# LuxGraph/Lux

Hardware: NVIDIA H100
Metric: MTEPS (higher is better)
Workload: dtype f32

## Files before the change

lux_b200/csrc/api.cu:

```cuda
#include <cub/cub.cuh>
#include <stdarg.h>
#include <stdlib.h>
#include <string.h>
#include <algorithm>
#include <type_traits>
#include <new>

#include "build.cuh"
#include "cf.cuh"
#include "pull.cuh"
#include "panel.cuh"
#include "seg.cuh"
#include "push.cuh"
#include "runtime.cuh"
#include <thrust/iterator/counting_iterator.h>

using namespace luxb;

enum class AppRun : uint8_t { kIterations, kConvergence, kEntry };
static constexpr char kBcRun[] = "luxb_bc_run";

struct AppInfo {
  const char* name;
  AppRun run;
  const char* entry;
  bool weights;
  bool dist_labels;
  uint32_t vbytes;
  bool check;
  bool settable;
};
static constexpr AppInfo kApps[] = {
    {"pagerank",                        AppRun::kIterations,  nullptr,          false,  false, 4,        false, true},
    {"connected components",            AppRun::kConvergence, nullptr,          false,  false, 4,        true,  true},
    {"SSSP",                            AppRun::kConvergence, nullptr,          false,  false, 4,        true,  true},
    {"col_filter",                      AppRun::kIterations,  nullptr,          true,   false, 4 * kCfK, false, true},
    {"weighted SSSP",                   AppRun::kConvergence, nullptr,          true,   true,  4,        true,  true},
    {"betweenness centrality",          AppRun::kEntry,       kBcRun,           false,  false, 8,        false, true},
    {"weighted betweenness centrality", AppRun::kEntry,       kBcRun,           true,   true,  8,        false, true},
    {"triangle counting",               AppRun::kEntry,       "luxb_tc_run",    false,  false, 8,        false, false},
    {"k-core decomposition",            AppRun::kEntry,       "luxb_kcore_run", false,  false, 4,        true,  true},
    {"k-truss decomposition",           AppRun::kEntry,       "luxb_truss_run", false,  false, 4,        true,  false},
};
static constexpr int kNumApps = sizeof(kApps) / sizeof(kApps[0]);
static_assert(kNumApps == LUXB_TRUSS + 1, "one row per luxb_app");
static const AppInfo& app_of(const luxb_graph* g) { return kApps[g->cfg.app]; }

static const char* const kPhaseName[12] = {"pull_tile", "fixup", "refresh", "rechunk", "barrier", "panel", "combine", "pack+push", "pull/bcast", "cold_hub", "bc_sigma", "bc_delta"};
static void pt_mark(luxb_graph* g, int tag) {
  PhaseTimer& pt = g->pt;
  if (!pt.on) return;
  cudaEvent_t e;
  cudaEventCreate(&e);
  cudaEventRecord(e, g->stream);
  pt.ev.push_back(e);
  pt.tag.push_back(tag);
}
static void pt_print(luxb_graph* g) {
  if (g->pt.on && g->pt.cnt) {
    char line[1024];
    const bool bc = app_of(g).entry == kBcRun;
    int n = snprintf(line, sizeof(line), "[luxb rank %d] phase means over %ld %s:", g->cfg.rank, g->pt.cnt, bc ? "sources" : "iterations");
    double sum = 0;
    for (int k = bc ? 10 : 0; k < (bc ? 12 : 10); ++k) {
      n += snprintf(line + n, sizeof(line) - n, " %s %.3f ms;", kPhaseName[k], g->pt.sum[k] / g->pt.cnt);
      sum += g->pt.sum[k] / g->pt.cnt;
    }
    snprintf(line + n, sizeof(line) - n, " sum %.3f ms\n", sum);
    fputs(line, stderr);
  }
}

static void pt_flush(luxb_graph* g) {
  PhaseTimer& pt = g->pt;
  if (!pt.on || pt.ev.empty()) return;
  cudaStreamSynchronize(g->stream);
  for (size_t i = 1; i < pt.ev.size(); ++i) {
    if (pt.tag[i] < 0) continue;
    float ms = 0;
    cudaEventElapsedTime(&ms, pt.ev[i - 1], pt.ev[i]);
    pt.sum[pt.tag[i]] += ms;
    if (pt.tag[i] == (app_of(g).entry == kBcRun ? 10 : 0)) pt.cnt++;
  }
  for (cudaEvent_t e : pt.ev) cudaEventDestroy(e);
  pt.ev.clear();
  pt.tag.clear();
}


namespace luxb {
static thread_local char g_err[1024] = "";
void set_error(const char* fmt, ...) {
  va_list ap;
  va_start(ap, fmt);
  vsnprintf(g_err, sizeof(g_err), fmt, ap);
  va_end(ap);
}
}

#define LUXB_ARG(cond, ...)             \
  do {                                  \
    if (!(cond)) {                      \
      set_error(__VA_ARGS__);           \
      return LUXB_ERR_ARG;              \
    }                                   \
  } while (0)

#define LUXB_NCCL(expr)                                                                              \
  do {                                                                                               \
    ncclResult_t _r = (expr);                                                                        \
    if (_r != ncclSuccess) {                                                                         \
      set_error("NCCL error %s at %s:%d: %s", #expr, __FILE__, __LINE__, nccl().GetErrorString(_r)); \
      return LUXB_ERR_COMM;                                                                          \
    }                                                                                                \
  } while (0)

#define LUXB_PULL_SHAPES(X) X(0, 7, 8, 2) X(1, 9, 8, 2) X(2, 7, 16, 2)
#define LUXB_DECL_SHAPE(id, ipt, warps, stages) using PullShape##id = PullShape<ipt, warps, stages>;
LUXB_PULL_SHAPES(LUXB_DECL_SHAPE)
// ... 785 lines not shown
      uint32_t zero = 0;
      if (start < g->nv)
        LUXB_CUDA(cudaMemcpyAsync(lab + start, &zero, 4, cudaMemcpyHostToDevice, g->stream));
    }
    LUXB_CUDA(cudaGetLastError());
  }
  if (g->n_part)
    LUXB_CUDA(cudaMemcpyAsync(g->d_cur, lab + g->row_left, (size_t)g->n_part * 4, cudaMemcpyDeviceToDevice, g->stream));
  LUXB_CUDA(cudaStreamSynchronize(g->stream));
  g->stats.last_active = 0;
  for (int p = 0; p < g->P; ++p) g->stats.last_active += g->h_hdr[2 * p + 1];
  g->stats.last_frontier_type = g->h_hdr[2 * g->cfg.rank];
  return 0;
}

static constexpr double kColdSplitWindowMB = 12.0;
static int set_l2_persisting_window(luxb_graph* g, void* base, size_t bytes) {
  if (!g->sweep.l2_persist) return 0;
  int max_persist = 0, max_window = 0;
  LUXB_CUDA(cudaDeviceGetAttribute(&max_persist, cudaDevAttrMaxPersistingL2CacheSize, g->cfg.device));
  LUXB_CUDA(cudaDeviceGetAttribute(&max_window, cudaDevAttrMaxAccessPolicyWindowSize, g->cfg.device));
  if (max_persist <= 0 || max_window <= 0) return 0;
  if (g->sweep.l2_window_mb >= 0) bytes = std::min<size_t>(bytes, (size_t)(g->sweep.l2_window_mb * 1e6));
  else if (g->cs_on) bytes = std::min<size_t>(bytes, (size_t)(kColdSplitWindowMB * 1e6));
  size_t persist = std::min<size_t>((size_t)max_persist, bytes);
  LUXB_CUDA(cudaDeviceSetLimit(cudaLimitPersistingL2CacheSize, persist));
  cudaStreamAttrValue attr{};
  attr.accessPolicyWindow.base_ptr = base;
  attr.accessPolicyWindow.num_bytes = std::min<size_t>(bytes, (size_t)max_window);
  attr.accessPolicyWindow.hitRatio = (float)std::min(1.0, (double)persist / (double)attr.accessPolicyWindow.num_bytes);
  attr.accessPolicyWindow.hitProp = cudaAccessPropertyPersisting;
  attr.accessPolicyWindow.missProp = cudaAccessPropertyStreaming;
  LUXB_CUDA(cudaStreamSetAttribute(g->stream, cudaStreamAttributeAccessPolicyWindow, &attr));
  if (g->cfg.verbose) printf("L2 persisting window: %zu bytes (device max persisting %d, max window %d)\n", persist, max_persist, max_window);
  return 0;
}

static constexpr double kColdSplitMinShare = 0.05;
static constexpr uint64_t kSplitMinEdges = 1ull << 24;

static bool split_may_run(const luxb_graph* g) {
  const SweepSettings& s = g->sweep;
  return s.seg && s.sb != 0 && !g->cfg.zero_copy_edges && (s.sb > 0 || g->e_part >= kSplitMinEdges);
}

static int build_hot_layout(luxb_graph* g, bool compact_cold) {
  g->hot_n = 0;
  g->packed = false;
  g->cold_z = false;
  uint64_t h_max = (uint64_t)(g->sweep.hot_mb * 1e6 / 4.0);
  if (h_max == 0 || g->nv < 2 || (uint64_t)g->nv >= 0xFFFFFFFFull - h_max) return 0;
  if (h_max > g->nv) h_max = g->nv;
  const int grid = g->num_sms * 8;
  const uint32_t cap = 4096;
  DevTmp tmp;
  unsigned long long* d_hist = nullptr;
  LUXB_TRY(tmp.alloc(&d_hist, cap + 1));
  LUXB_CUDA(cudaMemsetAsync(d_hist, 0, (cap + 1) * 8, g->stream));
  degree_hist_kernel<<<grid, 256, 0, g->stream>>>(g->d_deg, g->nv, cap, d_hist);
  std::vector<unsigned long long> hist(cap + 1);
  LUXB_CUDA(cudaMemcpyAsync(hist.data(), d_hist, (cap + 1) * 8, cudaMemcpyDeviceToHost, g->stream));
  LUXB_CUDA(cudaStreamSynchronize(g->stream));
  uint64_t above = 0;
  uint32_t tau = cap + 1;
  for (uint32_t d = cap; d >= 2; --d) {
    if (above + hist[d] > h_max) break;
// ... 88 lines not shown
    if (g->n_part)
      pack_list_cold_kernel<<<grid, 256, 0, g->stream>>>(d_cflag, d_crank, g->row_left, g->n_part, g->cold_off[me], g->d_pack_list + nh_me);
    LUXB_CUDA(cudaGetLastError());
    g->packed = true;
  }
  gather_map_hot_kernel<<<grid, 256, 0, g->stream>>>(d_map, g->d_hot_order, H);
  LUXB_TRY(edge_alloc(g, &g->d_src_gather, g->e_part + 8));
  LUXB_CUDA(cudaMemsetAsync(g->d_src_gather, 0, (g->e_part + 8) * 4, g->stream));
  remap_src_kernel<<<grid, 256, 0, g->stream>>>(g->d_src, g->e_part, d_map, g->d_src_gather);
  LUXB_CUDA(cudaGetLastError());
  LUXB_CUDA(cudaStreamSynchronize(g->stream));
  g->hot_n = H;
  return 0;
}

static int allgather_slices(luxb_graph* g, void* replica, size_t elem_bytes);
static void resolve_sweep_settings(SweepSettings& s);
static int build_seg_sweep(luxb_graph* g);
static int pagerank_publish(luxb_graph* g, float* x_new);
static int wait_cold_exchange(luxb_graph* g);
static int bc_alloc(luxb_graph* g);
static int tc_build(luxb_graph* g);
static int kcore_build(luxb_graph* g);
static int truss_build(luxb_graph* g);

static int build_gather_side(luxb_graph* g, bool compact_cold, bool streams) {
  LUXB_TRY(gmalloc(g, &g->d_deg, g->nv));
  LUXB_CUDA(cudaMemsetAsync(g->d_deg, 0, (size_t)g->nv * 4, g->stream));
  hist_src_kernel<<<g->num_sms * 8, 256, 0, g->stream>>>(g->d_src, g->e_part, g->d_deg);
  LUXB_CUDA(cudaGetLastError());
  if (g->P > 1) LUXB_NCCL(nccl().AllReduce(g->d_deg, g->d_deg, g->nv, ncclUint32, ncclSum, g->comm, g->stream));
  LUXB_TRY(build_hot_layout(g, compact_cold));
  if (streams) LUXB_TRY(build_seg_sweep(g));
  if (g->hot_n) {
    const uint64_t z_len = (uint64_t)g->hot_n + (g->cold_z ? g->cold_n : 0) + 65536;
    LUXB_TRY(gmalloc(g, (uint32_t**)&g->d_hot, z_len));
    LUXB_CUDA(cudaMemsetAsync(g->d_hot, 0, z_len * 4, g->stream));
    LUXB_TRY(set_l2_persisting_window(g, g->d_hot, (size_t)g->hot_n * 4));
  }
  return 0;
}

int luxb_init(luxb_graph* g) {
  LUXB_ARG(g != nullptr, "graph is NULL");
  if (g->inited) { set_error("luxb_init called twice"); return LUXB_ERR_STATE; }
  if (g->P > 1 && !g->comm) { set_error("luxb_init: nranks > 1 needs luxb_comm_init first"); return LUXB_ERR_STATE; }
  LUXB_CUDA(cudaSetDevice(g->cfg.device));
  resolve_sweep_settings(g->sweep);
  const int grid = g->num_sms * 8;
  switch (g->cfg.app) {
    case LUXB_PAGERANK: {
      LUXB_TRY(build_gather_side(g, true, true));
      for (int k = 0; k < 2; ++k) LUXB_TRY(gmalloc(g, (float**)&g->d_val[k], (uint64_t)g->nv + 64));
      pr_init_kernel<<<grid, 256, 0, g->stream>>>(g->d_deg, g->nv, (float*)g->d_val[0]);
      LUXB_CUDA(cudaMemsetAsync(g->d_val[1], 0, (size_t)g->nv * 4, g->stream));
      if (g->packed) {
        g->xt_hot_chunk = ((((uint64_t)g->hot_n + g->P - 1) / g->P) + 31) & ~31ull;
        g->xt_cold_chunk = ((((uint64_t)g->cold_n + g->P - 1) / g->P) + 31) & ~31ull;
        const uint64_t xt_len = (g->xt_hot_chunk + g->xt_cold_chunk) * g->P;
        for (int k = 0; k < 2; ++k) {
          LUXB_TRY(gmalloc(g, &g->d_xt[k], xt_len));
          LUXB_CUDA(cudaMemsetAsync(g->d_xt[k], 0, xt_len * 4, g->stream));
        }
      }
      LUXB_CUDA(cudaGetLastError());
      LUXB_TRY(pagerank_publish(g, (float*)g->d_val[0]));
// ... 109 lines not shown
  return 0;
}

static int kt_begin(luxb_graph* g) {
  if (!g->kernel_timing) return 0;
  if (g->kt_used + 2 > g->kt_events.size()) {
    cudaEvent_t e0, e1;
    LUXB_CUDA(cudaEventCreate(&e0));
    LUXB_CUDA(cudaEventCreate(&e1));
    g->kt_events.push_back(e0);
    g->kt_events.push_back(e1);
  }
  LUXB_CUDA(cudaEventRecord(g->kt_events[g->kt_used], g->stream));
  return 0;
}
static int kt_end(luxb_graph* g) {
  if (!g->kernel_timing) return 0;
  LUXB_CUDA(cudaEventRecord(g->kt_events[g->kt_used + 1], g->stream));
  g->kt_used += 2;
  return 0;
}

template <class Prog>
static void fill_fixup_args(PullArgs<Prog>& a, const FixupScratch& f) {
  a.head_partial = reinterpret_cast<typename Prog::Acc*>(f.d_head);
  a.tail_partial = reinterpret_cast<typename Prog::Acc*>(f.d_tail);
  a.carry = reinterpret_cast<typename Prog::Wide*>(f.d_carry);
  a.carry_flag = f.d_carry_flag;
  a.block_agg = reinterpret_cast<typename Prog::Wide*>(f.d_block_agg);
  a.block_flag = f.d_block_flag;
}

template <class Prog>
static int launch_fixup(luxb_graph* g, const PullArgs<Prog>& a, FixupScratch& f, const uint2* piece_slot = nullptr) {
  if (a.n_tiles <= 1) return 0;
  if (g->fused_fixup) {
    if (!f.d_chain) {
      LUXB_TRY(gmalloc(g, &f.d_chain, 4ull * f.n_fix_blocks + 4));
      LUXB_CUDA(cudaMemsetAsync(f.d_chain, 0, (4ull * f.n_fix_blocks + 4) * 8, g->stream));
      f.chain_epoch = 0;
    }
    FixupChain<Prog> ch;
    ch.value = f.d_chain;
    ch.status = f.d_chain + 2ull * f.n_fix_blocks;
    ch.ticket = f.d_chain + 4ull * f.n_fix_blocks;
    ch.n_blocks = f.n_fix_blocks;
    ch.epoch = ++f.chain_epoch;
    if (f.chain_epoch >= 0x3FFFFFF0u) {
      LUXB_CUDA(cudaMemsetAsync(f.d_chain, 0, (4ull * f.n_fix_blocks + 4) * 8, g->stream));
      f.chain_epoch = ch.epoch = 1;
    }
    pull_fixup_fused_kernel<Prog><<<f.n_fix_blocks, kFixBlock, 0, g->stream>>>(a, ch, piece_slot);
    LUXB_CUDA(cudaGetLastError());
    g->stats.kernel_launches++;
    return 0;
  }
  pull_fixup_scan_kernel<Prog><<<f.n_fix_blocks, kFixBlock, 0, g->stream>>>(a);
  pull_fixup_blocks_kernel<Prog><<<1, 1024, 0, g->stream>>>(a, f.n_fix_blocks);
  pull_fixup_apply_kernel<Prog><<<f.n_fix_blocks, kFixBlock, 0, g->stream>>>(a, piece_slot);
  LUXB_CUDA(cudaGetLastError());
  g->stats.kernel_launches += 3;
  return 0;
}

template <class Prog>
static int launch_pull(luxb_graph* g, PullLayout& L, const uint32_t* src, const typename Prog::Vertex* x_nat,
                       const typename Prog::Vertex* x_cold, const typename Prog::Vertex* x_hot, uint32_t hot_n,
                       typename Prog::Vertex* out_local, const typename Prog::Params& prm, const uint32_t* hub_bits = nullptr,
                       bool timed = true) {
  if (L.n_tiles == 0) return 0;
  PullArgs<Prog> a{};
  a.row_end = L.d_row_end;
  a.row_end32 = L.d_row_end32;
  a.src = src;
  a.x_nat = x_nat;
  a.n_part = L.n_vtx;
  a.e_part = L.e_cnt;
  a.row_left = g->row_left;
  a.x_old = x_cold;
  a.x_hot = x_hot;
  a.hot_n = hot_n;
  a.out = out_local;
  a.tile_v = L.d_tile_v;
  a.n_tiles = L.n_tiles;
  fill_fixup_args(a, L.fix);
  a.tile_counter = reinterpret_cast<uint32_t*>(g->d_counters + 2);
  LUXB_CUDA(cudaMemsetAsync(a.tile_counter, 0, 4, g->stream));
  a.prm = prm;
  a.hub_bits = hub_bits;
  a.raw_out = 0;
  if constexpr (Prog::kWeighted) a.weight = g->d_weight;
  if (timed) LUXB_TRY(kt_begin(g));
// ... 26 lines not shown
static const SegShapeInfo kSegPanelInfo[] = {LUXB_SEG_PANEL_SHAPES(LUXB_PSHAPE_INFO)};
static const int kNumSegMain = sizeof(kSegMainInfo) / sizeof(SegShapeInfo);
static const int kNumSegPanel = sizeof(kSegPanelInfo) / sizeof(SegShapeInfo);

static int env_int(const char* name, int dflt) {
  const char* e = getenv(name);
  return e ? atoi(e) : dflt;
}

static double env_double(const char* name, double dflt) {
  const char* e = getenv(name);
  return e ? atof(e) : dflt;
}

static void resolve_sweep_settings(SweepSettings& s) {
  s = SweepSettings();
  if (const char* e = getenv("LUXB_SWEEP")) s.seg = strcmp(e, "merge") != 0;
  auto shape = [](const char* name, int dflt, int n) { const int v = env_int(name, dflt); return v < 0 || v >= n ? 0 : v; };
  s.main_shape = shape("LUXB_SEG_MAIN_SHAPE", s.main_shape, kNumSegMain);
  s.panel_shape = shape("LUXB_SEG_PANEL_SHAPE", s.panel_shape, kNumSegPanel);
  s.cs_shape = shape("LUXB_CS_SHAPE", s.main_shape, kNumSegMain);
  s.sb = env_int("LUXB_SB", s.sb);
  const int tab = kSegPanelInfo[s.panel_shape].tab;
  s.sb_bs = std::min<uint32_t>((uint32_t)std::max(4, env_int("LUXB_SB_BS", tab)) & ~3u, (uint32_t)tab);
  s.sb_blocks = (uint32_t)std::min(std::max(env_int("LUXB_SB_BLOCKS", (int)s.sb_blocks), 1), kPanelMaxBlocks);
  s.sb_min_indeg = (uint32_t)std::max(env_int("LUXB_SB_MIN_INDEG", (int)s.sb_min_indeg), 1);
  s.sb_tier = env_int("LUXB_SB_TIER", s.sb_tier);
  s.sb_slot_edges = env_double("LUXB_SB_SLOT_EDGES", s.sb_slot_edges);
  s.cs = env_int("LUXB_CS", s.cs);
  s.cs_seg_mb = env_double("LUXB_CS_SEG_MB", s.cs_seg_mb);
  s.hot_mb = env_double("LUXB_HOT_MB", s.hot_mb);
  s.l2_persist = env_int("LUXB_L2_PERSIST", 1) != 0;
  s.l2_window_mb = env_double("LUXB_L2_WINDOW_MB", s.l2_window_mb);
}

extern "C++" {
template <class Word, class In>
static int build_seg_stream(luxb_graph* g, PullLayout& L, const uint64_t* d_row_end, uint32_t n_vtx, const In* d_ids, uint64_t e_cnt,
                            StreamBlocks& blk, uint32_t stage_edges, uint32_t piece, bool want_empty, const uint32_t* hub_bits,
                            uint32_t* super_end, bool slots = false, uint32_t slot_base = 0) {
  const int grid = g->num_sms * 8;
  DevTmp tmp;
  L = PullLayout();
  L.n_vtx = n_vtx;
  L.e_cnt = e_cnt;
  uint64_t words = 0, pads_total = 0;
  for (uint32_t b = 0; b < blk.n_blocks; ++b) {
    const uint64_t eb = blk.ebase[b + 1] - blk.ebase[b];
    const uint64_t pad = stage_edges - eb % stage_edges;
    blk.wbase[b] = words;
    blk.hshift[b] = pads_total;
    words += eb + pad;
    pads_total += pad;
    if (super_end) super_end[b] = (uint32_t)(words / stage_edges);
  }
  blk.wbase[blk.n_blocks] = words;
  blk.hshift[blk.n_blocks] = pads_total;
  LUXB_ARG(words / piece < 0xFFFFFFF0ull && words / stage_edges < 0xFFFFFFF0ull, "stream too large");
  L.n_words = words;
  L.n_stages = (uint32_t)(words / stage_edges);
  L.n_tiles = (uint32_t)(words / piece);
  uint32_t *d_flag = nullptr, *d_rank = nullptr;
  LUXB_TRY(tmp.alloc(&d_flag, (uint64_t)n_vtx + 1));
  LUXB_TRY(tmp.alloc(&d_rank, (uint64_t)n_vtx + 1));
  nonempty_flag_kernel<<<grid, 256, 0, g->stream>>>(d_row_end, n_vtx, d_flag);
  LUXB_CUDA(cudaMemsetAsync(d_flag + n_vtx, 0, 4, g->stream));
// ... 324 lines not shown
  g->stats.panel_edges = e_cov0;
  g->stats.panel_hubs = Nh;
  g->stats.panel_blocks = NB0;
  g->stats.cold_hub_edges = e_cold;
  g->stats.cold_hub_segments = S;
  g->stats.tier_blocks = NB - NB0;
  g->stats.tier_slots = NV - (uint64_t)NB0 * Nh;
  g->stats.tier_edges = e_cov - e_cov0;
  if (g->cfg.verbose) {
    printf("[luxb rank %d] source-blocked sweep: %u hub destinations (in-degree >= %u) x %u blocks of %u hot sources, + %u tier blocks "
           "(%llu slots, %llu edges); panel %llu edges (%.1f %%), cold-hub %llu edges (%u segments of %u values), main %llu edges\n",
           g->cfg.rank, Nh, st.sb_min_indeg, NB0, bs, NB - NB0, (unsigned long long)(NV - (uint64_t)NB0 * Nh), (unsigned long long)(e_cov - e_cov0),
           (unsigned long long)e_cov, 100.0 * e_cov / g->e_part, (unsigned long long)e_cold, S, cs.seg, (unsigned long long)e_main);
    printf("[luxb rank %d] (group, hub) pairs with edges / all: tier 0 %u / %llu, tiers %u / %llu, cold segments %u / %llu\n", g->cfg.rank,
           kind_slots[1], (unsigned long long)NB0 * Nh, kind_slots[2] - kind_slots[1], (unsigned long long)(NV - (uint64_t)NB0 * Nh),
           kind_slots[3] - kind_slots[2], (unsigned long long)Nh * S);
  }
  return 0;
}

static int build_seg_sweep(luxb_graph* g) {
  g->seg_on = false;
  g->sb_on = false;
  if (!g->sweep.seg) return 0;
  if (g->n_part == 0 || g->cfg.zero_copy_edges || g->e_part >= 0xFFFFFFF0ull) return 0;
  LUXB_TRY(build_panel_layout(g));
  if (!g->sb_on) LUXB_TRY(build_main_stream(g, g->d_row_end, g->hot_n ? g->d_src_gather : g->d_src, g->e_part, nullptr));
  g->seg_on = true;
  return 0;
}

extern "C++" {
template <class Prog, class Shape>
static int launch_seg_shape(luxb_graph* g, const SegArgs<Prog>& a, int ctas_per_sm) {
  auto kern = seg_tile_kernel<Prog, Shape>;
  const int reserve = (Shape::kPanel && g->packed) ? g->panel_reserve_sms : 0;
  LUXB_CUDA(cudaFuncSetAttribute(kern, cudaFuncAttributeMaxDynamicSharedMemorySize, (int)Shape::kSmemBytes));
  int carve_pct = (int)std::min<size_t>(100, (ctas_per_sm * (Shape::kSmemBytes + 1024) * 100 + 228 * 1024 - 1) / (228 * 1024));
  LUXB_CUDA(cudaFuncSetAttribute(kern, cudaFuncAttributePreferredSharedMemoryCarveout, carve_pct));
  const uint32_t grid = (uint32_t)std::min<uint64_t>((uint64_t)std::max(g->num_sms - reserve, 1) * ctas_per_sm, a.n_stages);
  kern<<<grid, Shape::kThreads, Shape::kSmemBytes, g->stream>>>(a);
  LUXB_CUDA(cudaGetLastError());
  return 0;
}

template <bool kPanel, class Prog, bool kSlots = kPanel>
static int launch_seg_stream(luxb_graph* g, PullLayout& L, SegArgs<Prog>& a, int shape, int ctas_per_sm, int counter_slot, int tag,
                             const char* name) {
  a.p.tile_v = L.d_tile_v;
  a.p.n_tiles = L.n_tiles;
  fill_fixup_args(a.p, L.fix);
  a.p.close_vtx = L.d_close;
  a.piece_slot = L.d_piece_slot;
  a.words = L.d_src;
  a.n_stages = L.n_stages;
  a.tile_counter = reinterpret_cast<uint32_t*>(g->d_counters + counter_slot);
  LUXB_CUDA(cudaMemsetAsync(a.tile_counter, 0, 4, g->stream));
#define LUXB_CASE_MSHAPE(id, warps, stages, rounds) \
  case id: LUXB_TRY((launch_seg_shape<Prog, std::conditional_t<kSlots, SlotShape<SegMain##id>, SegMain##id>>(g, a, ctas_per_sm))); break;
#define LUXB_CASE_PSHAPE(id, warps, stages, rounds, tab, v) \
  case id: LUXB_TRY((launch_seg_shape<Prog, SegPanel##id>(g, a, ctas_per_sm))); break;
  if constexpr (kPanel) {
    switch (shape) {
      LUXB_SEG_PANEL_SHAPES(LUXB_CASE_PSHAPE)
      default: set_error("bad %s shape", name); return LUXB_ERR_STATE;
    }
  } else {
    switch (shape) {
      LUXB_SEG_MAIN_SHAPES(LUXB_CASE_MSHAPE)
      default: set_error("bad %s shape", name); return LUXB_ERR_STATE;
    }
  }
  g->stats.kernel_launches++;
  pt_mark(g, tag);
  return launch_fixup(g, a.p, L.fix, L.d_piece_slot);
}
}

extern "C++" {
template <class Prog>
static int launch_seg_main(luxb_graph* g, PullLayout& L, const typename Prog::Vertex* x_nat, const typename Prog::Vertex* x_cold,
                           typename Prog::Vertex* out_local, int out_buffer, const typename Prog::Params& prm, const uint32_t* hub_bits) {
  SegArgs<Prog> a{};
  a.p.n_part = L.n_vtx;
  a.p.row_left = g->row_left;
  a.p.x_nat = x_nat;
  a.p.x_old = x_cold;
  a.p.x_hot = reinterpret_cast<const typename Prog::Vertex*>(g->d_hot);
  a.p.hot_n = g->hot_n;
  a.p.out = out_local;
  a.p.prm = prm;
  a.p.hub_bits = hub_bits;
  a.p.l2_hints = g->l2_hints;
  LUXB_TRY(wait_cold_exchange(g));
  LUXB_TRY((launch_seg_stream<false, Prog>(g, L, a, g->sweep.main_shape, g->pull_ctas, 2, 0, "seg")));
  if (out_buffer >= 0 && L.n_empty && !g->empties_done[out_buffer]) {
    empties_kernel<Prog><<<grid_for(L.n_empty, 256, g->num_sms * 8), 256, 0, g->stream>>>(a.p, L.d_empty, L.n_empty);
    g->empties_done[out_buffer] = true;
    g->stats.kernel_launches++;
  }
  if (L.n_empty_hub) {
    empties_kernel<Prog><<<grid_for(L.n_empty_hub, 256, g->num_sms * 8), 256, 0, g->stream>>>(a.p, L.d_empty_hub, L.n_empty_hub);
    g->stats.kernel_launches++;
  }
  LUXB_CUDA(cudaGetLastError());
  pt_mark(g, 1);
  return 0;
}

template <class Prog>
static int sweep_seg(luxb_graph* g, const typename Prog::Vertex* x_nat, const typename Prog::Vertex* x_cold, typename Prog::Vertex* out_local,
                     int out_buffer, const typename Prog::Params& prm) {
  using Acc = typename Prog::Acc;
  LUXB_TRY(kt_begin(g));
  if (g->sb_on) {
    SegArgs<Prog> pa{};
    pa.p.x_hot = reinterpret_cast<const typename Prog::Vertex*>(g->d_hot);
    pa.p.out = reinterpret_cast<typename Prog::Vertex*>(g->d_sb_partial);
    pa.p.raw_out = 1;
    pa.p.prm = prm;
    pa.bs = g->sb_bs;
    pa.n_blocks = g->sb_n_blocks;
    for (uint32_t b = 0; b < g->sb_n_blocks; ++b) pa.super_end[b] = g->sb_super_end[b];
    LUXB_TRY((launch_seg_stream<true, Prog>(g, g->sb_panel, pa, g->sweep.panel_shape, 1, 4, 5, "panel")));
    pt_mark(g, 1);
  }
  if (g->cs_on) {
    if constexpr (std::is_same<Prog, PageRankProgram>::value) {
      SegArgs<Prog> ca{};
      ca.p.x_old = x_cold;
      ca.p.x_hot = reinterpret_cast<const typename Prog::Vertex*>(g->d_hot);
      ca.p.hot_n = g->hot_n;
      ca.p.out = reinterpret_cast<typename Prog::Vertex*>(g->d_sb_partial);
      ca.p.raw_out = 1;
      ca.p.l2_hints = 0;
      ca.p.prm = prm;
      LUXB_TRY((launch_seg_stream<false, Prog, true>(g, g->sb_cold, ca, g->sweep.cs_shape, g->pull_ctas, 4, 9, "cold-hub")));
      pt_mark(g, 1);
    } else {
      set_error("the cold-hub stream is built for PageRank only");
      return LUXB_ERR_STATE;
    }
  }
  LUXB_TRY((launch_seg_main<Prog>(g, g->sb_main, x_nat, x_cold, out_local, out_buffer, prm, g->sb_on ? g->d_hub_bits : nullptr)));
  LUXB_TRY(kt_end(g));
  if (g->sb_on) {
    CombineArgs<Prog> ca{};
    ca.hub_vtx = g->d_hub_vtx;
    ca.n_hub = g->sb_n_hub;
    ca.n_blocks = g->sb_n_blocks;
    ca.n_groups = g->sb_n_groups;
    ca.row_left = g->row_left;
    ca.sg = g->sb_groups;
    ca.slot_bits = g->d_slot_bits;
    ca.slot_pre = g->d_slot_pre;
    ca.partial = reinterpret_cast<const Acc*>(g->d_sb_partial);
    ca.x_nat = x_nat;
    ca.out = out_local;
    ca.prm = prm;
    combine_hub_kernel<Prog><<<grid_for(g->sb_n_hub, 256, g->num_sms * 8), 256, 0, g->stream>>>(ca);
    LUXB_CUDA(cudaGetLastError());
    g->stats.kernel_launches++;
    pt_mark(g, 6);
  }
  return 0;
}
}

static int pagerank_publish(luxb_graph* g, float* x_new) {
  const int me = g->cfg.rank;
  const int grid = g->num_sms * 8;
  if (g->P == 1 || !g->packed) {
    if (g->P > 1) { LUXB_TRY(allgather_slices(g, x_new, 4)); pt_mark(g, 3); }
    if (g->hot_n) {
      const uint32_t z_n = g->hot_n + (g->cold_z ? g->cold_n : 0);
      hot_refresh_kernel<float><<<grid_for(z_n, 256, grid), 256, 0, g->stream>>>((float*)g->d_hot, x_new, g->d_hot_order, 0, z_n);
      LUXB_CUDA(cudaGetLastError());
      g->stats.kernel_launches++;
      pt_mark(g, 2);
    }
    return 0;
  }
  LUXB_TRY(wait_cold_exchange(g));
  float* XTn = g->d_xt[1 - g->cur_xt];
  const uint32_t H = g->hot_n;
  const uint64_t Ch = g->xt_hot_chunk, Cc = g->xt_cold_chunk, cold_base = Ch * g->P;
  const uint32_t nh_me = g->hot_off[me + 1] - g->hot_off[me], nc_me = g->cold_off[me + 1] - g->cold_off[me];
  const bool p2p = g->p2p_ready && g->cfg.exchange != LUXB_EXCHANGE_NCCL;
  if (p2p) {
    if (nh_me + nc_me) {
      PackPushArgs<float> pa{};
      pa.x_local = x_new + g->row_left;
      pa.list = g->d_pack_list;
// ... 340 lines not shown
      frontier_apply_kernel<<<grid_for(cnt, 256, g->num_sms * 4), 256, 0, g->stream>>>(slot_ptr(g->d_fq_all, g, p), g->cap[p], cnt, lab);
      g->stats.kernel_launches++;
    }
  }
  LUXB_CUDA(cudaGetLastError());
  g->stats.last_active = total;
  g->stats.last_frontier_type = my_hdr.type;
  g->trace_active.push_back(total);
  g->trace_pull.push_back(pull ? 1 : 0);
  if (g->cfg.verbose)
    printf("rowLeft(%u) activeNodes(%u) globalActive(%llu) %s\n", g->row_left, count, (unsigned long long)total, pull ? "pull" : "push");
  return 0;
}

}

static int one_iteration(luxb_graph* g) {
  switch (g->cfg.app) {
    case LUXB_PAGERANK: return pagerank_iteration(g);
    case LUXB_COLFILTER: return colfilter_iteration(g);
    case LUXB_CC: return label_iteration<MaxLabelProgram>(g);
    case LUXB_SSSP: return label_iteration<HopDistProgram>(g);
    case LUXB_SSSP_WEIGHTED: return label_iteration<WeightedDistProgram>(g);
  }
  return LUXB_ERR_ARG;
}

static int finish_timed(luxb_graph* g) {
  LUXB_TRY(wait_cold_exchange(g));
  pt_flush(g);
  if (g->pt.per_call) {
    pt_print(g);
    for (double& v : g->pt.sum) v = 0;
    g->pt.cnt = 0;
  }
  LUXB_CUDA(cudaEventRecord(g->ev_end, g->stream));
  LUXB_CUDA(cudaStreamSynchronize(g->stream));
  float ms = 0.f;
  LUXB_CUDA(cudaEventElapsedTime(&ms, g->ev_begin, g->ev_end));
  g->stats.loop_seconds += ms * 1e-3;
  if (g->h_barrier_err && *g->h_barrier_err) {
    set_error("iteration barrier: rank %u did not arrive within %llu s (LUXB_BARRIER_TIMEOUT_S)", *g->h_barrier_err - 1u,
              (unsigned long long)(g->barrier_timeout_ns / 1000000000ull));
    return LUXB_ERR_STATE;
  }
  for (size_t k = 0; k + 1 < g->kt_used; k += 2) {
    float kms = 0.f;
    LUXB_CUDA(cudaEventElapsedTime(&kms, g->kt_events[k], g->kt_events[k + 1]));
    g->stats.dominant_kernel_seconds += kms * 1e-3;
    g->stats.dominant_kernel_launches++;
  }
  g->kt_used = 0;
  if (g->d_out_end) {
    unsigned long long scanned = 0;
    LUXB_CUDA(cudaMemcpy(&scanned, g->d_counters, 8, cudaMemcpyDeviceToHost));
    LUXB_CUDA(cudaMemset(g->d_counters, 0, 8));
    g->stats.edges_processed += scanned;
  }
  return 0;
}

int luxb_iterate(luxb_graph* g, int iters, uint64_t* active_out) {
  LUXB_ARG(g != nullptr, "graph is NULL");
  if (!g->inited) { set_error("luxb_iterate before luxb_init"); return LUXB_ERR_STATE; }
  const AppInfo& app = app_of(g);
  LUXB_ARG(app.run != AppRun::kEntry, "luxb_iterate: %s runs through %s", app.name, app.entry);
// ... 1120 lines not shown
  out->row_right = g->row_left + g->n_part - 1;
  out->local_edges = g->e_part;
  return 0;
}

int luxb_get_local_csc(luxb_graph* g, luxb_eid* row_end_abs, luxb_vid* src, int32_t* weight) {
  LUXB_ARG(g != nullptr, "graph is NULL");
  LUXB_CUDA(cudaSetDevice(g->cfg.device));
  if (row_end_abs && g->n_part) {
    LUXB_CUDA(cudaMemcpy(row_end_abs, g->d_row_end, (size_t)g->n_part * 8, cudaMemcpyDeviceToHost));
    for (uint32_t i = 0; i < g->n_part; ++i) row_end_abs[i] += g->col_left;
  }
  if (src && g->e_part) LUXB_CUDA(cudaMemcpy(src, g->d_src, g->e_part * 4, cudaMemcpyDeviceToHost));
  if (weight) {
    LUXB_ARG(g->d_weight != nullptr, "graph has no weights");
    if (g->e_part) LUXB_CUDA(cudaMemcpy(weight, g->d_weight, g->e_part * 4, cudaMemcpyDeviceToHost));
  }
  return 0;
}

void luxb_close(luxb_graph* g) {
  if (!g) return;
  pt_print(g);
  cudaSetDevice(g->cfg.device);
  if (g->stream) cudaStreamSynchronize(g->stream);
  if (g->stream2) cudaStreamSynchronize(g->stream2);
  if (g->d_hot) cudaCtxResetPersistingL2Cache();
  p2p_unmap(g);
  if (g->stream2) cudaStreamSynchronize(g->stream2);
  if (g->comm) nccl().CommDestroy(g->comm);
  if (g->ev_pack) cudaEventDestroy(g->ev_pack);
  if (g->ev_cold) cudaEventDestroy(g->ev_cold);
  if (g->stream2) cudaStreamDestroy(g->stream2);
  for (size_t i = g->owned.size(); i-- > 0;) free_owned(g->owned[i]);
  for (cudaEvent_t e : g->kt_events) cudaEventDestroy(e);
  if (g->ev_begin) cudaEventDestroy(g->ev_begin);
  if (g->ev_end) cudaEventDestroy(g->ev_end);
  if (g->stream) cudaStreamDestroy(g->stream);
  delete g;
}

}
```

lux_b200/csrc/runtime.cuh:

```cuda
#pragma once
#include <vector>
#include "comm.h"
#include "common.cuh"
#include "panel.cuh"
#include "seg.cuh"
#include "push.cuh"
#include "bc.cuh"
#include "tc.cuh"
#include "kcore.cuh"
#include "truss.cuh"

struct FixupScratch {
  void* d_head = nullptr;
  void* d_tail = nullptr;
  void* d_carry = nullptr;
  uint32_t* d_carry_flag = nullptr;
  void* d_block_agg = nullptr;
  uint32_t* d_block_flag = nullptr;
  uint32_t n_fix_blocks = 0;
  unsigned long long* d_chain = nullptr;
  uint32_t chain_epoch = 0;
};

struct PullLayout {
  uint64_t* d_row_end = nullptr;
  uint32_t* d_row_end32 = nullptr;
  void* d_src = nullptr;
  uint32_t* d_tile_v = nullptr;
  uint32_t n_vtx = 0;
  uint64_t e_cnt = 0;
  uint32_t n_tiles = 0;
  FixupScratch fix;
  uint32_t* d_close = nullptr;
  uint2* d_piece_slot = nullptr;
  uint32_t n_slots = 0;
  uint32_t* d_empty = nullptr;
  uint32_t n_empty = 0;
  uint32_t* d_empty_hub = nullptr;
  uint32_t n_empty_hub = 0;
  uint32_t n_stages = 0;
  uint64_t n_words = 0;
};

struct SweepSettings {
  bool seg = true;
  int main_shape = 6, panel_shape = 1, cs_shape = 6;
  int sb = -1;
  uint32_t sb_bs = 0;
  uint32_t sb_blocks = 48;
  uint32_t sb_min_indeg = 64;
  int sb_tier = -1;
  double sb_slot_edges = 0.5;
  int cs = -1;
  double cs_seg_mb = 24.0;
  double hot_mb = 24.0;
  bool l2_persist = true;
  double l2_window_mb = -1.0;
};

struct PhaseTimer {
  bool on = false, per_call = false;
  std::vector<cudaEvent_t> ev;
  std::vector<int> tag;
  double sum[12] = {0};
  long cnt = 0;
};

struct CfState {
  uint32_t* chunk_first = nullptr;
  uint32_t* chunk_vtx = nullptr;
  uint32_t n_chunks = 0;
  float* partial = nullptr;
};

struct BcState {
  double* sigma = nullptr;
  double* delta = nullptr;
  double* scores = nullptr;
  uint32_t* order = nullptr;
  double* lvl = nullptr;
  uint64_t lvl_cap = 0;
  uint32_t* off = nullptr;
  uint64_t off_cap = 0;
  uint32_t* split = nullptr;
  uint64_t split_cap = 0;
  void* sort_tmp = nullptr;
  size_t sort_bytes = 0;
  uint32_t* ctl = nullptr;
  luxb::BcHub* hubs = nullptr;
  double* partial = nullptr;
  std::vector<uint32_t> h_off, h_split;
  bool has_source = false;
};

struct TcState {
  uint64_t m = 0;
  uint64_t* off = nullptr;
// ... 135 lines not shown
  TrussState tr;

  luxb::ncclComm_t comm = nullptr;
  bool p2p_ready = false;
  void* peer_val[2][LUXB_MAX_PARTS]{};
  void* peer_fq[LUXB_MAX_PARTS]{};
  uint32_t* d_sync = nullptr;
  uint32_t* d_flags = nullptr;
  void* peer_flags[LUXB_MAX_PARTS]{};
  uint32_t barrier_epoch = 0;
  uint32_t* h_barrier_err = nullptr;
  uint64_t barrier_timeout_ns = 30000000000ull;
  bool flag_barrier = true;
  bool flag_barrier_all = false;
  bool direct_push = false;

  SweepSettings sweep;

  bool empties_done[2] = {false, false};
  bool seg_on = false;
  bool sb_on = false;
  PullLayout sb_main, sb_panel;
  uint32_t sb_n_hub = 0, sb_n_blocks = 0, sb_n_groups = 0, sb_bs = 0;
  uint32_t* d_hub_vtx = nullptr;
  uint32_t* d_hub_bits = nullptr;
  uint32_t* d_sb_partial = nullptr;
  uint32_t* d_slot_bits = nullptr;
  uint32_t* d_slot_pre = nullptr;
  luxb::SplitGroups sb_groups{};
  uint32_t sb_super_end[luxb::kPanelMaxBlocks]{};
  bool cold_z = false;
  bool cs_on = false;
  PullLayout sb_cold;

  int pull_ctas = 3;
  bool overlap_exchange = true;
  bool fused_fixup = true;
  int panel_reserve_sms = 12;
  int l2_hints = 1;
  PhaseTimer pt;

  bool kernel_timing = false;
  std::vector<cudaEvent_t> kt_events;
  size_t kt_used = 0;

  std::vector<OwnedBuf> owned;

  luxb_stats_t stats{};
  std::vector<uint64_t> trace_active;
  std::vector<int32_t> trace_pull;
};
```

Before: 187,200.

## Run hub panel concurrently with main seg sweep on a second stream

```diff
diff --git a/lux_b200/csrc/api.cu b/lux_b200/csrc/api.cu
--- a/lux_b200/csrc/api.cu
+++ b/lux_b200/csrc/api.cu
@@ -46,7 +46,8 @@
 static_assert(kNumApps == LUXB_TRUSS + 1, "one row per luxb_app");
 static const AppInfo& app_of(const luxb_graph* g) { return kApps[g->cfg.app]; }
 
-static const char* const kPhaseName[12] = {"pull_tile", "fixup", "refresh", "rechunk", "barrier", "panel", "combine", "pack+push", "pull/bcast", "cold_hub", "bc_sigma", "bc_delta"};
+static const char* const kPhaseName[15] = {"pull_tile", "fixup", "refresh", "rechunk", "barrier", "panel", "combine", "pack+push",
+                                           "pull/bcast", "cold_hub", "bc_sigma", "bc_delta", "main_join", "join_wait", "overlap"};
 static void pt_mark(luxb_graph* g, int tag) {
   PhaseTimer& pt = g->pt;
   if (!pt.on) return;
@@ -55,6 +56,18 @@
   cudaEventRecord(e, g->stream);
   pt.ev.push_back(e);
   pt.tag.push_back(tag);
+}
+static int pt_event(luxb_graph* g, cudaStream_t st) {
+  PhaseTimer& pt = g->pt;
+  if (!pt.on) return -1;
+  cudaEvent_t e;
+  cudaEventCreate(&e);
+  cudaEventRecord(e, st);
+  pt.span_ev.push_back(e);
+  return (int)pt.span_ev.size() - 1;
+}
+static void pt_span(luxb_graph* g, int tag, int begin, int end) {
+  if (begin >= 0) g->pt.spans.push_back({begin, end, tag});
 }
 static void pt_print(luxb_graph* g) {
   if (g->pt.on && g->pt.cnt) {
@@ -66,6 +79,10 @@
       n += snprintf(line + n, sizeof(line) - n, " %s %.3f ms;", kPhaseName[k], g->pt.sum[k] / g->pt.cnt);
       sum += g->pt.sum[k] / g->pt.cnt;
     }
+    if (!bc && g->pt.sum[14] > 0) {
+      for (int k = 12; k < 15; ++k) n += snprintf(line + n, sizeof(line) - n, " %s %.3f ms;", kPhaseName[k], g->pt.sum[k] / g->pt.cnt);
+      sum = g->pt.chain / g->pt.cnt;
+    }
     snprintf(line + n, sizeof(line) - n, " sum %.3f ms\n", sum);
     fputs(line, stderr);
   }
@@ -75,16 +92,27 @@
   PhaseTimer& pt = g->pt;
   if (!pt.on || pt.ev.empty()) return;
   cudaStreamSynchronize(g->stream);
+  const int count_tag = app_of(g).entry == kBcRun ? 10 : 0;
   for (size_t i = 1; i < pt.ev.size(); ++i) {
     if (pt.tag[i] < 0) continue;
     float ms = 0;
     cudaEventElapsedTime(&ms, pt.ev[i - 1], pt.ev[i]);
     pt.sum[pt.tag[i]] += ms;
-    if (pt.tag[i] == (app_of(g).entry == kBcRun ? 10 : 0)) pt.cnt++;
+    pt.chain += ms;
+    if (pt.tag[i] == count_tag) pt.cnt++;
+  }
+  for (const PhaseTimer::Span& s : pt.spans) {
+    float ms = 0;
+    cudaEventElapsedTime(&ms, pt.span_ev[s.begin], pt.span_ev[s.end]);
+    pt.sum[s.tag] += ms;
+    if (s.tag == count_tag) pt.cnt++;
   }
   for (cudaEvent_t e : pt.ev) cudaEventDestroy(e);
+  for (cudaEvent_t e : pt.span_ev) cudaEventDestroy(e);
   pt.ev.clear();
   pt.tag.clear();
+  pt.span_ev.clear();
+  pt.spans.clear();
 }
 
 
@@ -936,6 +964,7 @@
   attr.accessPolicyWindow.hitProp = cudaAccessPropertyPersisting;
   attr.accessPolicyWindow.missProp = cudaAccessPropertyStreaming;
   LUXB_CUDA(cudaStreamSetAttribute(g->stream, cudaStreamAttributeAccessPolicyWindow, &attr));
+  if (g->stream_b) LUXB_CUDA(cudaStreamSetAttribute(g->stream_b, cudaStreamAttributeAccessPolicyWindow, &attr));
   if (g->cfg.verbose) printf("L2 persisting window: %zu bytes (device max persisting %d, max window %d)\n", persist, max_persist, max_window);
   return 0;
 }
@@ -1090,6 +1119,11 @@
   if (g->P > 1) LUXB_NCCL(nccl().AllReduce(g->d_deg, g->d_deg, g->nv, ncclUint32, ncclSum, g->comm, g->stream));
   LUXB_TRY(build_hot_layout(g, compact_cold));
   if (streams) LUXB_TRY(build_seg_sweep(g));
+  if (g->sb_on && g->P == 1) {
+    LUXB_CUDA(cudaStreamCreateWithFlags(&g->stream_b, cudaStreamNonBlocking));
+    LUXB_CUDA(cudaEventCreateWithFlags(&g->ev_fork, cudaEventDisableTiming));
+    LUXB_CUDA(cudaEventCreateWithFlags(&g->ev_join, cudaEventDisableTiming));
+  }
   if (g->hot_n) {
     const uint64_t z_len = (uint64_t)g->hot_n + (g->cold_z ? g->cold_n : 0) + 65536;
     LUXB_TRY(gmalloc(g, (uint32_t**)&g->d_hot, z_len));
@@ -1265,12 +1299,14 @@
 }
 
 template <class Prog>
-static int launch_fixup(luxb_graph* g, const PullArgs<Prog>& a, FixupScratch& f, const uint2* piece_slot = nullptr) {
+static int launch_fixup(luxb_graph* g, const PullArgs<Prog>& a, FixupScratch& f, const uint2* piece_slot = nullptr,
+                        cudaStream_t st = nullptr) {
   if (a.n_tiles <= 1) return 0;
+  if (!st) st = g->stream;
   if (g->fused_fixup) {
     if (!f.d_chain) {
       LUXB_TRY(gmalloc(g, &f.d_chain, 4ull * f.n_fix_blocks + 4));
-      LUXB_CUDA(cudaMemsetAsync(f.d_chain, 0, (4ull * f.n_fix_blocks + 4) * 8, g->stream));
+      LUXB_CUDA(cudaMemsetAsync(f.d_chain, 0, (4ull * f.n_fix_blocks + 4) * 8, st));
       f.chain_epoch = 0;
     }
     FixupChain<Prog> ch;
@@ -1280,17 +1316,17 @@
     ch.n_blocks = f.n_fix_blocks;
     ch.epoch = ++f.chain_epoch;
     if (f.chain_epoch >= 0x3FFFFFF0u) {
-      LUXB_CUDA(cudaMemsetAsync(f.d_chain, 0, (4ull * f.n_fix_blocks + 4) * 8, g->stream));
+      LUXB_CUDA(cudaMemsetAsync(f.d_chain, 0, (4ull * f.n_fix_blocks + 4) * 8, st));
       f.chain_epoch = ch.epoch = 1;
     }
-    pull_fixup_fused_kernel<Prog><<<f.n_fix_blocks, kFixBlock, 0, g->stream>>>(a, ch, piece_slot);
+    pull_fixup_fused_kernel<Prog><<<f.n_fix_blocks, kFixBlock, 0, st>>>(a, ch, piece_slot);
     LUXB_CUDA(cudaGetLastError());
     g->stats.kernel_launches++;
     return 0;
   }
-  pull_fixup_scan_kernel<Prog><<<f.n_fix_blocks, kFixBlock, 0, g->stream>>>(a);
-  pull_fixup_blocks_kernel<Prog><<<1, 1024, 0, g->stream>>>(a, f.n_fix_blocks);
-  pull_fixup_apply_kernel<Prog><<<f.n_fix_blocks, kFixBlock, 0, g->stream>>>(a, piece_slot);
+  pull_fixup_scan_kernel<Prog><<<f.n_fix_blocks, kFixBlock, 0, st>>>(a);
+  pull_fixup_blocks_kernel<Prog><<<1, 1024, 0, st>>>(a, f.n_fix_blocks);
+  pull_fixup_apply_kernel<Prog><<<f.n_fix_blocks, kFixBlock, 0, st>>>(a, piece_slot);
   LUXB_CUDA(cudaGetLastError());
   g->stats.kernel_launches += 3;
   return 0;
@@ -1383,6 +1419,7 @@
   s.hot_mb = env_double("LUXB_HOT_MB", s.hot_mb);
   s.l2_persist = env_int("LUXB_L2_PERSIST", 1) != 0;
   s.l2_window_mb = env_double("LUXB_L2_WINDOW_MB", s.l2_window_mb);
+  s.panel_sms = std::max(0, env_int("LUXB_PANEL_SMS", s.panel_sms));
 }
 
 extern "C++" {
@@ -1773,21 +1810,20 @@
 
 extern "C++" {
 template <class Prog, class Shape>
-static int launch_seg_shape(luxb_graph* g, const SegArgs<Prog>& a, int ctas_per_sm) {
+static int launch_seg_shape(luxb_graph* g, const SegArgs<Prog>& a, int sms, int ctas_per_sm, cudaStream_t st) {
   auto kern = seg_tile_kernel<Prog, Shape>;
   const int reserve = (Shape::kPanel && g->packed) ? g->panel_reserve_sms : 0;
   LUXB_CUDA(cudaFuncSetAttribute(kern, cudaFuncAttributeMaxDynamicSharedMemorySize, (int)Shape::kSmemBytes));
   int carve_pct = (int)std::min<size_t>(100, (ctas_per_sm * (Shape::kSmemBytes + 1024) * 100 + 228 * 1024 - 1) / (228 * 1024));
   LUXB_CUDA(cudaFuncSetAttribute(kern, cudaFuncAttributePreferredSharedMemoryCarveout, carve_pct));
-  const uint32_t grid = (uint32_t)std::min<uint64_t>((uint64_t)std::max(g->num_sms - reserve, 1) * ctas_per_sm, a.n_stages);
-  kern<<<grid, Shape::kThreads, Shape::kSmemBytes, g->stream>>>(a);
-  LUXB_CUDA(cudaGetLastError());
-  return 0;
-}
-
-template <bool kPanel, class Prog, bool kSlots = kPanel>
-static int launch_seg_stream(luxb_graph* g, PullLayout& L, SegArgs<Prog>& a, int shape, int ctas_per_sm, int counter_slot, int tag,
-                             const char* name) {
+  const uint32_t grid = (uint32_t)std::min<uint64_t>((uint64_t)std::max(std::min(sms, g->num_sms - reserve), 1) * ctas_per_sm, a.n_stages);
+  kern<<<grid, Shape::kThreads, Shape::kSmemBytes, st>>>(a);
+  LUXB_CUDA(cudaGetLastError());
+  return 0;
+}
+
+template <class Prog>
+static void seg_stream_args(luxb_graph* g, PullLayout& L, SegArgs<Prog>& a, int counter_slot) {
   a.p.tile_v = L.d_tile_v;
   a.p.n_tiles = L.n_tiles;
   fill_fixup_args(a.p, L.fix);
@@ -1796,11 +1832,15 @@
   a.words = L.d_src;
   a.n_stages = L.n_stages;
   a.tile_counter = reinterpret_cast<uint32_t*>(g->d_counters + counter_slot);
-  LUXB_CUDA(cudaMemsetAsync(a.tile_counter, 0, 4, g->stream));
+}
+
+template <bool kPanel, class Prog, bool kSlots = kPanel>
+static int launch_seg_kernel(luxb_graph* g, const SegArgs<Prog>& a, int shape, int sms, int ctas_per_sm, cudaStream_t st,
+                             const char* name) {
 #define LUXB_CASE_MSHAPE(id, warps, stages, rounds) \
-  case id: LUXB_TRY((launch_seg_shape<Prog, std::conditional_t<kSlots, SlotShape<SegMain##id>, SegMain##id>>(g, a, ctas_per_sm))); break;
+  case id: LUXB_TRY((launch_seg_shape<Prog, std::conditional_t<kSlots, SlotShape<SegMain##id>, SegMain##id>>(g, a, sms, ctas_per_sm, st))); break;
 #define LUXB_CASE_PSHAPE(id, warps, stages, rounds, tab, v) \
-  case id: LUXB_TRY((launch_seg_shape<Prog, SegPanel##id>(g, a, ctas_per_sm))); break;
+  case id: LUXB_TRY((launch_seg_shape<Prog, SegPanel##id>(g, a, sms, ctas_per_sm, st))); break;
   if constexpr (kPanel) {
     switch (shape) {
       LUXB_SEG_PANEL_SHAPES(LUXB_CASE_PSHAPE)
@@ -1813,6 +1853,12 @@
     }
   }
   g->stats.kernel_launches++;
+  return 0;
+}
+
+template <bool kPanel, class Prog, bool kSlots = kPanel>
+static int launch_seg_stream(luxb_graph* g, PullLayout& L, const SegArgs<Prog>& a, int shape, int ctas_per_sm, int tag, const char* name) {
+  LUXB_TRY((launch_seg_kernel<kPanel, Prog, kSlots>(g, a, shape, g->num_sms, ctas_per_sm, g->stream, name)));
   pt_mark(g, tag);
   return launch_fixup(g, a.p, L.fix, L.d_piece_slot);
 }
@@ -1820,8 +1866,8 @@
 
 extern "C++" {
 template <class Prog>
-static int launch_seg_main(luxb_graph* g, PullLayout& L, const typename Prog::Vertex* x_nat, const typename Prog::Vertex* x_cold,
-                           typename Prog::Vertex* out_local, int out_buffer, const typename Prog::Params& prm, const uint32_t* hub_bits) {
+static SegArgs<Prog> seg_main_args(luxb_graph* g, PullLayout& L, const typename Prog::Vertex* x_nat, const typename Prog::Vertex* x_cold,
+                                   typename Prog::Vertex* out_local, const typename Prog::Params& prm, const uint32_t* hub_bits) {
   SegArgs<Prog> a{};
   a.p.n_part = L.n_vtx;
   a.p.row_left = g->row_left;
@@ -1833,19 +1879,22 @@
   a.p.prm = prm;
   a.p.hub_bits = hub_bits;
   a.p.l2_hints = g->l2_hints;
-  LUXB_TRY(wait_cold_exchange(g));
-  LUXB_TRY((launch_seg_stream<false, Prog>(g, L, a, g->sweep.main_shape, g->pull_ctas, 2, 0, "seg")));
+  seg_stream_args(g, L, a, 2);
+  return a;
+}
+
+template <class Prog>
+static int launch_seg_empties(luxb_graph* g, PullLayout& L, const PullArgs<Prog>& p, int out_buffer) {
   if (out_buffer >= 0 && L.n_empty && !g->empties_done[out_buffer]) {
-    empties_kernel<Prog><<<grid_for(L.n_empty, 256, g->num_sms * 8), 256, 0, g->stream>>>(a.p, L.d_empty, L.n_empty);
+    empties_kernel<Prog><<<grid_for(L.n_empty, 256, g->num_sms * 8), 256, 0, g->stream>>>(p, L.d_empty, L.n_empty);
     g->empties_done[out_buffer] = true;
     g->stats.kernel_launches++;
   }
   if (L.n_empty_hub) {
-    empties_kernel<Prog><<<grid_for(L.n_empty_hub, 256, g->num_sms * 8), 256, 0, g->stream>>>(a.p, L.d_empty_hub, L.n_empty_hub);
+    empties_kernel<Prog><<<grid_for(L.n_empty_hub, 256, g->num_sms * 8), 256, 0, g->stream>>>(p, L.d_empty_hub, L.n_empty_hub);
     g->stats.kernel_launches++;
   }
   LUXB_CUDA(cudaGetLastError());
-  pt_mark(g, 1);
   return 0;
 }
 
@@ -1853,9 +1902,9 @@
 static int sweep_seg(luxb_graph* g, const typename Prog::Vertex* x_nat, const typename Prog::Vertex* x_cold, typename Prog::Vertex* out_local,
                      int out_buffer, const typename Prog::Params& prm) {
   using Acc = typename Prog::Acc;
-  LUXB_TRY(kt_begin(g));
+  constexpr bool kColdHub = std::is_same<Prog, PageRankProgram>::value;
+  SegArgs<Prog> pa{}, ca{};
   if (g->sb_on) {
-    SegArgs<Prog> pa{};
     pa.p.x_hot = reinterpret_cast<const typename Prog::Vertex*>(g->d_hot);
     pa.p.out = reinterpret_cast<typename Prog::Vertex*>(g->d_sb_partial);
     pa.p.raw_out = 1;
@@ -1863,12 +1912,10 @@
     pa.bs = g->sb_bs;
     pa.n_blocks = g->sb_n_blocks;
     for (uint32_t b = 0; b < g->sb_n_blocks; ++b) pa.super_end[b] = g->sb_super_end[b];
-    LUXB_TRY((launch_seg_stream<true, Prog>(g, g->sb_panel, pa, g->sweep.panel_shape, 1, 4, 5, "panel")));
-    pt_mark(g, 1);
+    seg_stream_args(g, g->sb_panel, pa, 4);
   }
   if (g->cs_on) {
-    if constexpr (std::is_same<Prog, PageRankProgram>::value) {
-      SegArgs<Prog> ca{};
+    if constexpr (kColdHub) {
       ca.p.x_old = x_cold;
       ca.p.x_hot = reinterpret_cast<const typename Prog::Vertex*>(g->d_hot);
       ca.p.hot_n = g->hot_n;
@@ -1876,30 +1923,80 @@
       ca.p.raw_out = 1;
       ca.p.l2_hints = 0;
       ca.p.prm = prm;
-      LUXB_TRY((launch_seg_stream<false, Prog, true>(g, g->sb_cold, ca, g->sweep.cs_shape, g->pull_ctas, 4, 9, "cold-hub")));
-      pt_mark(g, 1);
+      seg_stream_args(g, g->sb_cold, ca, 5);
     } else {
       set_error("the cold-hub stream is built for PageRank only");
       return LUXB_ERR_STATE;
     }
   }
-  LUXB_TRY((launch_seg_main<Prog>(g, g->sb_main, x_nat, x_cold, out_local, out_buffer, prm, g->sb_on ? g->d_hub_bits : nullptr)));
+  const SegArgs<Prog> ma = seg_main_args<Prog>(g, g->sb_main, x_nat, x_cold, out_local, prm, g->sb_on ? g->d_hub_bits : nullptr);
+  const int S = g->sweep.panel_sms;
+  const bool beside = g->stream_b && S > 0 && S < g->num_sms;
+  LUXB_TRY(kt_begin(g));
+  LUXB_CUDA(cudaMemsetAsync(g->d_counters + 2, 0, 4, g->stream));
+  if (g->sb_on) LUXB_CUDA(cudaMemsetAsync(g->d_counters + 4, 0, 16, g->stream));
+  if (beside) {
+    cudaStream_t sb = g->stream_b;
+    LUXB_CUDA(cudaEventRecord(g->ev_fork, g->stream));
+    const int t_fork = pt_event(g, g->stream);
+    LUXB_TRY((launch_seg_kernel<true, Prog>(g, pa, g->sweep.panel_shape, S, 1, g->stream, "panel")));
+    pt_mark(g, 5);
+    LUXB_CUDA(cudaStreamWaitEvent(sb, g->ev_fork, 0));
+    int t = pt_event(g, sb);
+    if constexpr (kColdHub) {
+      if (g->cs_on) {
+        LUXB_TRY((launch_seg_kernel<false, Prog, true>(g, ca, g->sweep.cs_shape, g->num_sms - S, g->pull_ctas, sb, "cold-hub")));
+        const int t_cold = pt_event(g, sb);
+        pt_span(g, 9, t, t_cold);
+        LUXB_TRY(launch_fixup(g, ca.p, g->sb_cold.fix, g->sb_cold.d_piece_slot, sb));
+        t = pt_event(g, sb);
+        pt_span(g, 1, t_cold, t);
+      }
+    }
+    LUXB_TRY((launch_seg_kernel<false, Prog>(g, ma, g->sweep.main_shape, g->num_sms - S, g->pull_ctas, sb, "seg")));
+    pt_span(g, 0, t, pt_event(g, sb));
+    LUXB_CUDA(cudaEventRecord(g->ev_join, sb));
+    LUXB_TRY(launch_fixup(g, pa.p, g->sb_panel.fix, g->sb_panel.d_piece_slot));
+    pt_mark(g, 1);
+    LUXB_TRY((launch_seg_kernel<false, Prog>(g, ma, g->sweep.main_shape, S, g->pull_ctas, g->stream, "seg")));
+    pt_mark(g, 12);
+    LUXB_CUDA(cudaStreamWaitEvent(g->stream, g->ev_join, 0));
+    pt_mark(g, 13);
+    pt_span(g, 14, t_fork, pt_event(g, g->stream));
+  } else {
+    if (g->sb_on) {
+      LUXB_TRY((launch_seg_stream<true, Prog>(g, g->sb_panel, pa, g->sweep.panel_shape, 1, 5, "panel")));
+      pt_mark(g, 1);
+    }
+    if constexpr (kColdHub) {
+      if (g->cs_on) {
+        LUXB_TRY((launch_seg_stream<false, Prog, true>(g, g->sb_cold, ca, g->sweep.cs_shape, g->pull_ctas, 9, "cold-hub")));
+        pt_mark(g, 1);
+      }
+    }
+    LUXB_TRY(wait_cold_exchange(g));
+    LUXB_TRY((launch_seg_kernel<false, Prog>(g, ma, g->sweep.main_shape, g->num_sms, g->pull_ctas, g->stream, "seg")));
+    pt_mark(g, 0);
+  }
+  LUXB_TRY(launch_fixup(g, ma.p, g->sb_main.fix, g->sb_main.d_piece_slot));
+  LUXB_TRY(launch_seg_empties(g, g->sb_main, ma.p, out_buffer));
+  pt_mark(g, 1);
   LUXB_TRY(kt_end(g));
   if (g->sb_on) {
-    CombineArgs<Prog> ca{};
-    ca.hub_vtx = g->d_hub_vtx;
-    ca.n_hub = g->sb_n_hub;
-    ca.n_blocks = g->sb_n_blocks;
-    ca.n_groups = g->sb_n_groups;
-    ca.row_left = g->row_left;
-    ca.sg = g->sb_groups;
-    ca.slot_bits = g->d_slot_bits;
-    ca.slot_pre = g->d_slot_pre;
-    ca.partial = reinterpret_cast<const Acc*>(g->d_sb_partial);
-    ca.x_nat = x_nat;
-    ca.out = out_local;
-    ca.prm = prm;
-    combine_hub_kernel<Prog><<<grid_for(g->sb_n_hub, 256, g->num_sms * 8), 256, 0, g->stream>>>(ca);
+    CombineArgs<Prog> cb{};
+    cb.hub_vtx = g->d_hub_vtx;
+    cb.n_hub = g->sb_n_hub;
+    cb.n_blocks = g->sb_n_blocks;
+    cb.n_groups = g->sb_n_groups;
+    cb.row_left = g->row_left;
+    cb.sg = g->sb_groups;
+    cb.slot_bits = g->d_slot_bits;
+    cb.slot_pre = g->d_slot_pre;
+    cb.partial = reinterpret_cast<const Acc*>(g->d_sb_partial);
+    cb.x_nat = x_nat;
+    cb.out = out_local;
+    cb.prm = prm;
+    combine_hub_kernel<Prog><<<grid_for(g->sb_n_hub, 256, g->num_sms * 8), 256, 0, g->stream>>>(cb);
     LUXB_CUDA(cudaGetLastError());
     g->stats.kernel_launches++;
     pt_mark(g, 6);
@@ -2306,6 +2403,7 @@
   if (g->pt.per_call) {
     pt_print(g);
     for (double& v : g->pt.sum) v = 0;
+    g->pt.chain = 0;
     g->pt.cnt = 0;
   }
   LUXB_CUDA(cudaEventRecord(g->ev_end, g->stream));
@@ -3492,6 +3590,9 @@
   if (g->ev_pack) cudaEventDestroy(g->ev_pack);
   if (g->ev_cold) cudaEventDestroy(g->ev_cold);
   if (g->stream2) cudaStreamDestroy(g->stream2);
+  if (g->ev_fork) cudaEventDestroy(g->ev_fork);
+  if (g->ev_join) cudaEventDestroy(g->ev_join);
+  if (g->stream_b) cudaStreamDestroy(g->stream_b);
   for (size_t i = g->owned.size(); i-- > 0;) free_owned(g->owned[i]);
   for (cudaEvent_t e : g->kt_events) cudaEventDestroy(e);
   if (g->ev_begin) cudaEventDestroy(g->ev_begin);
diff --git a/lux_b200/csrc/runtime.cuh b/lux_b200/csrc/runtime.cuh
--- a/lux_b200/csrc/runtime.cuh
+++ b/lux_b200/csrc/runtime.cuh
@@ -56,13 +56,18 @@
   double hot_mb = 24.0;
   bool l2_persist = true;
   double l2_window_mb = -1.0;
+  int panel_sms = 40;
 };
 
 struct PhaseTimer {
+  struct Span { int begin, end, tag; };
   bool on = false, per_call = false;
   std::vector<cudaEvent_t> ev;
   std::vector<int> tag;
-  double sum[12] = {0};
+  std::vector<cudaEvent_t> span_ev;
+  std::vector<Span> spans;
+  double sum[15] = {0};
+  double chain = 0;
   long cnt = 0;
 };
 
@@ -264,6 +269,8 @@
   bool cold_z = false;
   bool cs_on = false;
   PullLayout sb_cold;
+  cudaStream_t stream_b = nullptr;
+  cudaEvent_t ev_fork = nullptr, ev_join = nullptr;
 
   int pull_ctas = 3;
   bool overlap_exchange = true;
```

New measurement: 212,700, median of 6. 13.7% higher.
